# dexmal/dexbotic

Measured on AMD Instinct MI355X. Metric: episodes/sec DB-CogACT fine-tune, higher is better.
Workload: dtype bf16; 1 GPU; DB-CogACT fine-tune step (CLIP-L/14@224 x1 view, Qwen2.5-7B-class 28L decoder, DiT-B head, AdamW), 16 episodes/GPU, 32-token instruction, S=287; global_batch=16, seq_len=287, parallelism=dp1, optimizer=AdamW serial, grad_accum=1, activations=resident

## Files before the change

dexbotic_amd/_lib.py:

```python
from __future__ import annotations

import ctypes as C
import os

import torch

_HERE = os.path.dirname(os.path.abspath(__file__))
LIB_PATH = os.environ.get("DXA_LIB") or os.path.join(_HERE, "libdexbotic_amd.so")

F32, BF16 = 0, 1
ACT_NONE, ACT_GELU_ERF, ACT_GELU_TANH, ACT_QUICK_GELU, ACT_SILU, ACT_RELU, ACT_SIGMOID = 0, 1, 2, 3, 4, 5, 6
NT, NN, TN = 0, 1, 2
FILTER_BICUBIC = 3
FUSE_NONE, FUSE_SWIGLU = 0, 1

_vp, _i64, _i32, _f32, _sz = C.c_void_p, C.c_int64, C.c_int32, C.c_float, C.c_size_t
_int = C.c_int


class DxaError(RuntimeError):
    pass


class GemmDesc(C.Structure):
    _fields_ = [
        ("layout", _i32), ("in_dtype", _i32), ("out_dtype", _i32), ("act", _i32),
        ("M", _i64), ("N", _i64), ("K", _i64),
        ("A", _vp), ("lda", _i64), ("B", _vp), ("ldb", _i64), ("C", _vp), ("ldc", _i64),
        ("bias", _vp), ("residual", _vp), ("ldr", _i64), ("aux_out", _vp), ("mulgrad", _vp), ("ldg", _i64),
        ("alpha", _f32), ("accumulate", _i32), ("nb", _i32 * 3),
        ("sA", _i64 * 3), ("sB", _i64 * 3), ("sC", _i64 * 3), ("sR", _i64 * 3), ("sG", _i64 * 3),
        ("epi_f32", _i32), ("mirror", _vp), ("sumsq", _vp),
        ("A2", _vp), ("B2", _vp), ("K2", _i64),
        ("fuse", _i32), ("ld_aux", _i64),
    ]


class GemmStepInfo(C.Structure):
    _fields_ = [
        ("kernel", C.c_char_p), ("grid", _i32 * 3), ("block", _i32), ("lds", _i32),
        ("K", _i64), ("K2", _i64), ("a_off", _i64), ("b_off", _i64), ("seg2", _i32),
        ("accumulate", _i32), ("bias", _i32), ("residual", _i32),
        ("tm", _i32), ("tn", _i32), ("full", _i32), ("tail_r", _i32), ("split_s", _i32), ("group_m", _i32),
        ("vecA", _i32), ("vecB", _i32), ("vecC", _i32), ("vecR", _i32), ("vecG", _i32), ("vecBias", _i32),
        ("ksplit", _i32), ("kper", _i32), ("split_ws", _i32), ("mirror", _i32), ("sumsq", _i32),
    ]

# ... 32 lines not shown
        ("beta1", _f32), ("beta2", _f32), ("eps", _f32), ("bc1", _f32), ("bc2", _f32),
        ("clip_coef", _vp), ("g_dtype", _i32), ("chunk_state", _vp), ("chunk_mv_start", _vp),
    ]


class ImageDesc(C.Structure):
    _fields_ = [
        ("src", _vp), ("n", _i32), ("h", _i32), ("w", _i32), ("pad", _i32), ("bg", C.c_ubyte * 4),
        ("res_h", _i32), ("res_w", _i32), ("crop_top", _i32), ("crop_left", _i32), ("out_h", _i32), ("out_w", _i32),
        ("row0", _i32), ("rows", _i32), ("hb", _vp), ("hk", _vp), ("hks", _i32), ("vb", _vp), ("vk", _vp), ("vks", _i32),
        ("tmp", _vp), ("out", _vp), ("out_dtype", _i32), ("out_u8", _vp), ("rescale", C.c_double),
        ("mean", _f32 * 3), ("std", _f32 * 3),
    ]


class DecodeDesc(C.Structure):
    _fields_ = [
        ("layers", _vp), ("x_in", _vp), ("out", _vp), ("final_norm_w", _vp), ("cos_row", _vp), ("sin_row", _vp),
        ("workspace", _vp), ("workspace_bytes", _sz),
        ("n_layers", _i32), ("d", _i32), ("Hq", _i32), ("Hkv", _i32), ("D", _i32), ("F", _i32), ("slot", _i32), ("kv_lo", _i32),
        ("max_len", _i32), ("eps", _f32),
    ]


SIGNATURES = {
    "dxa_last_error": (C.c_char_p, []),
    "dxa_version": (_int, []),
    "dxa_gemm": (_int, [C.POINTER(GemmDesc), _vp]),
    "dxa_gemm_plan": (_int, [C.POINTER(GemmDesc), C.POINTER(GemmPlanInfo)]),
    "dxa_gemm_kernel_name": (C.c_char_p, [_int]),
    "dxa_split3": (_int, [_vp, _i64, _vp, _i64, _i64, _int, _vp]),
    "dxa_split3_t": (_int, [_vp, _i64, _vp, _i64, _i64, _i64, _int, _vp]),
    "dxa_split3_pair": (_int, [C.POINTER(Split3Op), C.POINTER(Split3Op), _vp]),
    "dxa_rmsnorm_fwd": (_int, [_vp, _vp, _vp, _vp, _i64, _i64, _f32, _int, _int, _vp]),
    "dxa_rmsnorm_bwd": (_int, [_vp, _vp, _vp, _vp, _vp, _vp, _vp, _i64, _i64, _int, _int, _vp]),
    "dxa_layernorm_fwd": (_int, [_vp, _vp, _vp, _vp, _vp, _vp, _i64, _i64, _f32, _int, _int, _vp]),
    "dxa_layernorm_bwd": (_int, [_vp, _vp, _vp, _vp, _vp, _vp, _vp, _vp, _i64, _i64, _int, _int, _vp]),
    "dxa_norm_bwd_blocks": (_int, [_i64]),
    "dxa_colsum": (_int, [_vp, _i64, _vp, _i64, _i64, _int, _int, _vp, _sz, _vp]),
    "dxa_rope_split": (_int, [_vp, _vp, _vp, _vp, _vp, _vp, _vp, _int, _int, _int, _int, _int, _int, _vp]),
    "dxa_rope_merge": (_int, [_vp, _vp, _vp, _vp, _vp, _vp, _vp, _int, _int, _int, _int, _int, _int, _vp]),
    "dxa_rope_split_at": (_int, [_vp, _vp, _vp, _vp, _vp, _vp, _vp, _int, _int, _int, _int, _int, _int, _int, _int, _vp]),
    "dxa_rope_merge_at": (_int, [_vp, _vp, _vp, _vp, _vp, _vp, _vp, _int, _int, _int, _int, _int, _int, _int, _int, _vp]),
    "dxa_attn_fwd": (_int, [C.POINTER(AttnDesc), _vp]),
    "dxa_attn_fwd_workspace": (_sz, [C.POINTER(AttnDesc)]),
    "dxa_attn_fwd_ws": (_int, [C.POINTER(AttnDesc), _vp, _sz, _vp]),
    "dxa_attn_bwd_workspace": (_sz, [C.POINTER(AttnDesc)]),
    "dxa_attn_bwd": (_int, [C.POINTER(AttnDesc), _vp, _sz, _vp]),
    "dxa_swiglu_fwd": (_int, [_vp, _vp, _i64, _i64, _int, _vp]),
    "dxa_swiglu_bwd": (_int, [_vp, _vp, _vp, _i64, _i64, _int, _vp]),
    "dxa_axpby": (_int, [_vp, _vp, _vp, _i64, _f32, _f32, _int, _vp]),
    "dxa_mul": (_int, [_vp, _vp, _vp, _i64, _int, _vp]),
    "dxa_mul_rows": (_int, [_vp, _vp, _vp, _i64, _i64, _i64, _int, _vp]),
    "dxa_glu_fwd": (_int, [_vp, _vp, _i64, _i64, _int, _int, _vp]),
    "dxa_glu_bwd": (_int, [_vp, _vp, _vp, _i64, _i64, _int, _int, _vp]),
    "dxa_act_fwd": (_int, [_vp, _vp, _i64, _int, _int, _vp]),
    "dxa_act_bwd": (_int, [_vp, _vp, _vp, _i64, _int, _int, _vp]),
    "dxa_add": (_int, [_vp, _vp, _vp, _i64, _int, _vp]),
    "dxa_cast": (_int, [_vp, _vp, _i64, _int, _int, _vp]),
    "dxa_copy2d": (_int, [_vp, _i64, _vp, _i64, _i64, _i64, _i64, _int, _int, _vp]),
    "dxa_transpose": (_int, [_vp, _i64, _vp, _i64, _i64, _i64, _i64, _int, _vp]),
    "dxa_permute_bshd": (_int, [_vp, _vp, _int, _int, _int, _int, _int, _int, _vp]),
    "dxa_splice_fwd": (_int, [_vp, _vp, _vp, _vp, _i64, _i64, _int, _vp]),
    "dxa_splice_bwd": (_int, [_vp, _vp, _vp, _vp, _i64, _i64, _int, _vp]),
    "dxa_zero_rows": (_int, [_vp, _vp, _i64, _i64, _vp]),
    "dxa_gather_rows": (_int, [_vp, _vp, _vp, _i64, _i64, _int, _int, _vp]),
# ... 77 lines not shown
```

dexbotic_amd/csrc/gemm.hip:

```cpp
#include "common.h"
#include "gemm_common.h"

#include <algorithm>
#include <cassert>

namespace {


template <typename T> struct EltTraits;
template <> struct EltTraits<float> { static constexpr int EPC = 4; };
template <> struct EltTraits<bf16_t> { static constexpr int EPC = 8; };

__device__ __forceinline__ int lds_off(int row, int chunk) { return row * ROWB + ((chunk ^ (row & 7)) << 4); }

template <typename T, int NR>
__device__ __forceinline__ void load_kc(uint4 (&r)[4], const T* __restrict__ base, int64_t ld, int64_t row0,
                                        int64_t rows, int64_t k0, int64_t K, int vec, int tid) {
  constexpr int EPC = EltTraits<T>::EPC;
  const int c = tid & 7;
  const int64_t k = k0 + (int64_t)c * EPC;
#pragma unroll
  for (int i = 0; i < NR / 32; ++i) {
    const int64_t row = row0 + (tid >> 3) + 32 * i;
    uint4 v = make_uint4(0, 0, 0, 0);
// ... 1213 lines not shown
  if (wm == 0) P3_BAR();
  P3_STAMP(2);
#undef P3_A_ROW0
#undef P3_B_ROW0
#undef P3_DMA
#undef P3_DMA_A
#undef P3_DMA_B
#undef P3_READ
#undef P3_RD_A
#undef P3_RD_B
#undef P3_MFMA
#undef P3_SB
#undef P3_BAR
#undef P3_COMPUTE
#undef P3_VMCNT
#undef P3_TILE
#undef P3_R_A1
#undef P3_R_A2B0
#undef P3_R_A0B1
  if constexpr (LEAN) {
    if (!tile_split_exchange<3>(p, acc, tid, split_j, split_s, tail_i)) return;
    __builtin_amdgcn_sched_barrier(0);
    if constexpr (FUSE == 1) sk_epilogue_swiglu<3>(p, acc, smem + wave * 4096, lane, wm, wn, (int)m0, (int)n0);
    else sk_epilogue<TO, TE, 3>(p, acc, smem + wave * 4096, lane, wm, wn, (int)m0, (int)n0, reinterpret_cast<float*>(smem + 8 * 4096), bid);
  } else {
    tile_finish<TO, 3, TE>(p, acc, smem, tid, lane, wave, wm, wn, l32, lh, m0, n0, split_j, split_s, tail_i);
  }
  asm volatile("s_waitcnt vmcnt(0)" ::: "memory");
  P3_STAMP(3);
#endif
}
#undef P3_STAMP

template <typename T>
__global__ __launch_bounds__(256) void sumsq_rows_k(const T* __restrict__ C, int64_t ldc, int64_t M, int64_t N,
                                                    float* __restrict__ out) {
  __shared__ float red[4];
  float s = 0.f;
  for (int64_t r = blockIdx.x; r < M; r += gridDim.x) {
    const T* row = C + r * ldc;
    for (int64_t c = threadIdx.x; c < N; c += 256) { const float v = ldf<T>(row + c); s += v * v; }
  }
#pragma unroll
  for (int o = 32; o > 0; o >>= 1) s += __shfl_xor(s, o, 64);
  if ((threadIdx.x & 63) == 0) red[threadIdx.x >> 6] = s;
  __syncthreads();
  if (threadIdx.x == 0) out[blockIdx.x] = (red[0] + red[1]) + (red[2] + red[3]);
}


constexpr int NUM_CU = 256;
static_assert(NUM_CU == NUM_CU_D, "split-K scratch sizing");
constexpr size_t SPLIT_WS_BYTES = (size_t)NUM_CU * 256 * 256 * 4;
int get_split_ws(hipStream_t st, char** ws) {
  static StreamBlock blocks(SPLIT_WS_BYTES + NUM_CU * sizeof(int));
  char* base = nullptr;
  if (int rc = blocks.get(st, &base)) return rc;
  DXA_CHECK_ARG(base != nullptr, "dxa_gemm: first split-K product on a stream allocates its scratch and cannot happen under stream "
                "capture: run the request once eagerly on this stream first");
  *ws = base;
  return DXA_OK;
}

enum GemmArgs { ARGS_P, ARGS_GEMV1, ARGS_GEMV2 };
struct GemmKernel {
  const char* name;
// ... 260 lines not shown
  p.C = (char*)d->C; p.ldc = d->ldc;
  p.bias = s.bias ? (const char*)d->bias : nullptr;
  p.R = s.residual ? (const char*)d->residual : nullptr; p.ldr = d->ldr;
  p.aux = (char*)d->aux_out;
  p.G = (const char*)d->mulgrad; p.ldg = d->ldg;
  p.alpha = d->alpha; p.act = d->act; p.accumulate = s.accumulate;
  p.fuse = d->fuse; p.ldaux = d->ld_aux;
  p.nb1 = d->nb[1]; p.nb2 = d->nb[2];
  for (int i = 0; i < 3; ++i) {
    p.sA[i] = d->sA[i]; p.sB[i] = d->sB[i]; p.sC[i] = d->sC[i]; p.sR[i] = d->sR[i]; p.sG[i] = d->sG[i];
  }
  p.tm = s.tm; p.tn = s.tn;
  p.vecA = s.vecA; p.vecB = s.vecB; p.vecC = s.vecC; p.vecR = s.vecR; p.vecG = s.vecG; p.vecBias = s.vecBias;
  p.full = s.full; p.tail_r = s.tail_r; p.split_s = s.split_s; p.group_m = s.group_m;
  if (s.mirror) p.mirror = (char*)d->mirror;
  if (s.sumsq) p.sumsq = d->sumsq;
  if (s.K2 > 0) { p.A2 = (const char*)d->A2; p.B2 = (const char*)d->B2; p.K2 = s.K2; }
  if (s.split_ws) {
    if (*ws == nullptr)
      if (int rc = get_split_ws(st, ws)) return rc;
    p.ws = (float*)*ws; p.flags = (int*)(*ws + SPLIT_WS_BYTES);
  }
  if (int rc = k.raise ? k.raise(k.lds) : DXA_OK) return rc;
  int M = (int)d->M, ksplit = s.ksplit, kper = s.kper;
  void* args_p[] = {&p};
  void* args_gemv1[] = {&p.A, &p.lda, &p.B, &p.ldb, &p.ws, &M, &p.N, &p.K, &kper};
  void* args_gemv2[] = {&p.ws, &p.C, &p.ldc, &M, &p.N, &ksplit, &p.alpha};
  void** args = k.args == ARGS_P ? args_p : k.args == ARGS_GEMV1 ? args_gemv1 : args_gemv2;
  (void)hipLaunchKernel(k.fn, dim3(s.grid[0], s.grid[1], s.grid[2]), dim3(k.block), args, k.lds, st);
  DXA_CHECK_LAUNCH();
  return DXA_OK;
}

}

extern "C" int64_t dxa_gemm_sumsq_slots(int64_t M, int64_t N) {
  if (M <= 0 || N <= 0) return 0;
  return ((M + 255) / 256) * ((N + 255) / 256);
}
extern "C" const char* dxa_gemm_kernel_name(int i) {
  return i >= 0 && i < NUM_KERNELS ? reinterpret_cast<const GemmKernel*>(&KERNELS)[i].name : nullptr;
}
extern "C" int dxa_gemm_plan(const dxa_gemm_desc* d, dxa_gemm_plan_info* out) {
  DXA_CHECK_ARG(out != nullptr, "dxa_gemm_plan: null output");
  GemmPlan plan;
  const int rc = gemm_plan(d, &plan);
  *out = plan.info;
  return rc;
}
extern "C" int dxa_gemm(const dxa_gemm_desc* d, dxa_stream_t stream) {
  GemmPlan plan;
  if (int rc = gemm_plan(d, &plan)) return rc;
  char* ws = nullptr;
  for (int i = 0; i < plan.info.nsteps; ++i) {
    if (int rc = gemm_run_step(d, plan.info.step[i], *plan.kernel[i], (hipStream_t)stream, &ws)) return rc;
  }
  if (plan.info.mirror_pass) {
    if (int rc = dxa_copy2d(d->C, d->ldc, d->mirror, d->ldc, d->M, d->N, d->N, DXA_F32, DXA_BF16, stream)) return rc;
  }
  if (plan.info.sumsq_pass) {
    const dim3 sgrid((unsigned)dxa_gemm_sumsq_slots(d->M, d->N));
    if (d->out_dtype == DXA_F32)
      hipLaunchKernelGGL(sumsq_rows_k<float>, sgrid, dim3(256), 0, (hipStream_t)stream, (const float*)d->C, d->ldc, d->M, d->N, d->sumsq);
    else
      hipLaunchKernelGGL(sumsq_rows_k<bf16_t>, sgrid, dim3(256), 0, (hipStream_t)stream, (const bf16_t*)d->C, d->ldc, d->M, d->N, d->sumsq);
    DXA_CHECK_LAUNCH();
  }
  return DXA_OK;
}

namespace {
struct S3Op { const float* src; int64_t ld; bf16_t* dst; int64_t rows, cols, pad; int side, transposed; unsigned nblocks, tiles_x; };
__global__ __launch_bounds__(256) void split3_pair_k(const S3Op a, const S3Op b) {
  __shared__ float tile[32][33];
  const bool first = blockIdx.x < a.nblocks;
  const S3Op& o = first ? a : b;
  const unsigned bid = first ? blockIdx.x : blockIdx.x - a.nblocks;
  if (!o.transposed) {
    const int64_t c4 = o.cols >> 2;
    for (int64_t i = (int64_t)bid * 256 + threadIdx.x; i < o.rows * c4; i += (int64_t)o.nblocks * 256) {
      const int64_t r = i / c4, c = (i - r * c4) * 4;
      float x[4];
      Vec<float, 4>::ld(x, o.src + r * o.ld + c);
      float hi[4], lo[4];
#pragma unroll
      for (int e = 0; e < 4; ++e) {
        hi[e] = bf2f(f2bf(x[e]));
        lo[e] = x[e] - hi[e];
      }
      bf16_t* d = o.dst + r * 3 * o.cols + c;
      Vec<bf16_t, 4>::st(d, hi);
      Vec<bf16_t, 4>::st(d + o.cols, o.side == 0 ? hi : lo);
      Vec<bf16_t, 4>::st(d + 2 * o.cols, o.side == 0 ? lo : hi);
    }
    return;
  }
  const int tx = threadIdx.x & 31, ty = threadIdx.x >> 5;
  const int64_t R = o.rows, C_ = o.cols, Rp = o.pad;
  const int64_t r0 = (int64_t)(bid / o.tiles_x) * 32, c0 = (int64_t)(bid % o.tiles_x) * 32;
#pragma unroll
  for (int i = 0; i < 4; ++i) {
// ... 75 lines not shown
```

dexbotic_amd/csrc/gemm_common.h:

```cpp
#pragma once
#include "common.h"

namespace dxa_gemm_detail {
typedef float f32x16_t __attribute__((ext_vector_type(16)));
struct GemmP {
  int64_t M, N, K;
  const char* A; int64_t lda;
  const char* B; int64_t ldb;
  char* C; int64_t ldc;
  const char* bias;
  const char* R; int64_t ldr;
  char* aux;
  const char* G; int64_t ldg;
  float alpha;
  int act, accumulate;
  int nb1, nb2;
  int64_t sA[3], sB[3], sC[3], sR[3], sG[3];
  int tm, tn;
  int vecA, vecB, vecC, vecR, vecG, vecBias;
  int full, tail_r, split_s;
  int group_m;
  char* mirror;
  float* sumsq;
  float* ws;
// ... 490 lines not shown
          const u32x2_t_ gv = {pack_bf16x2(g[0], g[1]), pack_bf16x2(g[2], g[3])};
          const u32x2_t_ uv = {pack_bf16x2(u[0], u[1]), pack_bf16x2(u[2], u[3])};
          __builtin_amdgcn_raw_buffer_store_b64(gv, rX, ok ? offG0 + rr * ldxB : 0x80000000u, 0, 0);
          __builtin_amdgcn_raw_buffer_store_b64(uv, rX, ok ? offU0 + rr * ldxB : 0x80000000u, 0, 0);
        }
      }
      __builtin_amdgcn_fence(__ATOMIC_RELEASE, "wavefront");
      __builtin_amdgcn_wave_barrier();
      __builtin_amdgcn_sched_barrier(0);
    }
#endif
}
template <typename TO, typename TE, int AI = 4, int MF = 32>
__device__ __forceinline__ void sk_epilogue(const GemmP& p, typename AccL<AI, MF>::T& acc, char* slab, int lane, int wm, int wn,
                                            int m0, int n0, float* red, int tile) {
#if defined(__HIP_DEVICE_COMPILE__)
  float ssq = sk_epilogue_rows<TO, TE, AI, MF>(p, acc, slab, lane, wm, wn, m0, n0);
  {
    if (p.sumsq != nullptr) {
#pragma unroll
      for (int o = 32; o > 0; o >>= 1) ssq += __shfl_xor(ssq, o, 64);
      if (lane == 0) red[wm * 4 + wn] = ssq;
      __syncthreads();
      if (threadIdx.x == 0) {
        float t = 0.f;
#pragma unroll
        for (int w8 = 0; w8 < 8; ++w8) t += red[w8];
        p.sumsq[tile] = t;
      }
    }
  }
#endif
}
}
```

dexbotic_amd/kernels.py:

```python
from __future__ import annotations

import contextlib
import ctypes as C
from typing import Optional, Sequence, Tuple

import torch

from . import _lib as L
from ._lib import lib

F32, BF16 = L.F32, L.BF16


def dt(t: torch.Tensor) -> int:
    if t.dtype == torch.float32:
        return F32
    if t.dtype == torch.bfloat16:
        return BF16
    raise L.DxaError(f"unsupported dtype {t.dtype} (fp32 / bf16 only)")


def torch_dtype(code: int) -> torch.dtype:
    return torch.bfloat16 if code == BF16 else torch.float32

# ... 52 lines not shown
    return out


def split3_pair(a: torch.Tensor, a_t: bool, b: torch.Tensor, b_t: bool, pad_to: int = 1, a_dims=None, b_dims=None
                ) -> Tuple[torch.Tensor, torch.Tensor]:
    ops, outs = [], []
    for x, t, side, dims in ((a, a_t, 0, a_dims), (b, b_t, 1, b_dims)):
        R, C_, ld = dims if dims is not None else (x.shape[0], x.shape[1], _row_major(x, "x"))
        o = L.Split3Op()
        o.src, o.ld, o.rows, o.cols, o.side, o.transposed = _ptr(x), ld, R, C_, side, int(t)
        if t:
            Rp = (R + pad_to - 1) // pad_to * pad_to
            out = torch.empty((C_, 3 * Rp), device=x.device, dtype=torch.bfloat16)
            o.pad = Rp
        else:
            out = torch.empty((R, 3 * C_), device=x.device, dtype=torch.bfloat16)
            o.pad = 0
        o.dst = _ptr(out)
        ops.append(o)
        outs.append(out)
    L.check(lib.dxa_split3_pair(C.byref(ops[0]), C.byref(ops[1]), _stream()), "dxa_split3_pair")
    return outs[0], outs[1]


def _x3_t_ok(M: int, N: int, Kc: int, out: torch.Tensor) -> bool:
    return (F32_GEMM_MODE == "bf16x3" and out.dtype == torch.float32 and M >= 128 and N >= 128 and Kc >= 64 and Kc % 32 == 0
            and 6 * max(M, N) * Kc < (1 << 31))


def mm_tn_f32(a: torch.Tensor, b: torch.Tensor, *, out: torch.Tensor, **kw) -> torch.Tensor:
    Kc, M = a.shape
    N = b.shape[1]
    if a.dtype == torch.float32 and b.dtype == torch.float32 and _x3_t_ok(M, N, (Kc + 31) // 32 * 32, out):
        a3, b3 = split3_pair(a, True, b, True, pad_to=32)
        Kp = a3.shape[1] // 3
        kw = _ld_kwargs(kw, out)
        return gemm(L.NT, a3, b3, M, N, 3 * Kp, 3 * Kp, 3 * Kp, out, _row_major(out, "out"), epi_f32=True, **kw)
    return mm_nt(transpose(a, 4), transpose(b, 4), out=out, **kw)


def mm_nn_f32(a: torch.Tensor, b: torch.Tensor, **kw) -> torch.Tensor:
    M, Kc = a.shape
    N = b.shape[1]
    out = kw.get("out")
    if (a.dtype == torch.float32 and b.dtype == torch.float32 and Kc % 32 == 0 and a.is_contiguous() and a.data_ptr() % 16 == 0
            and Kc % 4 == 0 and (out is None or out.dtype == torch.float32)):
        if out is None:
            out = kw["out"] = torch.empty((M, N), device=a.device, dtype=torch.float32)
        if _x3_t_ok(M, N, Kc, out):
            a3, b3 = split3_pair(a, False, b, True)
            kw2 = _ld_kwargs({k: v for k, v in kw.items() if k != "out"}, out)
            return gemm(L.NT, a3, b3, M, N, 3 * Kc, 3 * Kc, 3 * Kc, out, _row_major(out, "out"), epi_f32=True, **kw2)
    return mm_nt(a, transpose(b, 1), **kw)


def _x3_eligible(layout, a, b, out, M, N, K, lda, ldb, nb) -> bool:
    return (F32_GEMM_MODE == "bf16x3" and layout == L.NT and a.dtype == torch.float32 and b.dtype == torch.float32
            and out.dtype == torch.float32 and tuple(nb) == (1, 1, 1) and M >= 128 and N >= 128 and K >= 64 and K % 32 == 0
            and lda % 4 == 0 and ldb % 4 == 0 and a.data_ptr() % 16 == 0 and b.data_ptr() % 16 == 0
            and 6 * max(M, N) * K < (1 << 31))


_NB1 = (1, 1, 1)


def gemm(layout: int, a: torch.Tensor, b: torch.Tensor, M: int, N: int, K: int, lda: int, ldb: int,
         out: torch.Tensor, ldc: int, *, bias: Optional[torch.Tensor] = None,
         residual: Optional[torch.Tensor] = None, ldr: int = 0, act: int = L.ACT_NONE,
         aux_out: Optional[torch.Tensor] = None, mulgrad: Optional[torch.Tensor] = None, ldg: int = 0,
         alpha: float = 1.0, accumulate: bool = False, nb: Sequence[int] = _NB1,
         sA: Sequence[int] = (0, 0, 0), sB: Sequence[int] = (0, 0, 0), sC: Sequence[int] = (0, 0, 0),
         sR: Sequence[int] = (0, 0, 0), sG: Sequence[int] = (0, 0, 0), epi_f32: bool = False,
         mirror: Optional[torch.Tensor] = None, sumsq: Optional[torch.Tensor] = None,
         a2: Optional[torch.Tensor] = None, b2: Optional[torch.Tensor] = None) -> torch.Tensor:
    if not epi_f32 and a2 is None and _x3_eligible(layout, a, b, out, M, N, K, lda, ldb, nb):
        a3, b3 = split3_pair(a, False, b, False, a_dims=(M, K, lda), b_dims=(N, K, ldb))
        return gemm(L.NT, a3, b3, M, N, 3 * K, 3 * K, 3 * K, out, ldc, bias=bias, residual=residual, ldr=ldr, act=act,
                    aux_out=aux_out, mulgrad=mulgrad, ldg=ldg, alpha=alpha, accumulate=accumulate, epi_f32=True,
                    mirror=mirror, sumsq=sumsq)
    d = L.GemmDesc()
    d.layout, d.in_dtype, d.out_dtype, d.act = layout, dt(a), dt(out), act
    d.epi_f32 = int(epi_f32)
    if dt(b) != d.in_dtype:
        raise L.DxaError("gemm: A and B dtypes differ")
    for t, n in ((bias, "bias"), (residual, "residual"), (mulgrad, "mulgrad")):
        if t is not None and dt(t) != (F32 if epi_f32 else d.in_dtype):
            raise L.DxaError(f"gemm: {n} dtype must equal the input dtype")
    if aux_out is not None and dt(aux_out) != d.out_dtype:
        raise L.DxaError("gemm: aux_out dtype must equal the output dtype")
    d.M, d.N, d.K = M, N, K
    d.A, d.lda, d.B, d.ldb, d.C, d.ldc = _ptr(a), lda, _ptr(b), ldb, _ptr(out), ldc
    d.bias, d.residual, d.ldr = _ptr(bias), _ptr(residual), ldr
    d.aux_out, d.mulgrad, d.ldg = _ptr(aux_out), _ptr(mulgrad), ldg
    d.alpha, d.accumulate = alpha, int(accumulate)
    if mirror is not None:
        if mirror.dtype != torch.bfloat16 or out.dtype != torch.float32 or tuple(nb) != (1, 1, 1) or \
                _row_major(mirror, "mirror") != ldc:
            raise L.DxaError("gemm: mirror must be a bf16 [M, N] view with the output's leading dimension (fp32 output)")
        d.mirror = _ptr(mirror)
    if sumsq is not None:
        if sumsq.dtype != torch.float32 or tuple(nb) != (1, 1, 1) or not sumsq.is_contiguous() \
                or sumsq.numel() != gemm_sumsq_slots(M, N):
            raise L.DxaError("gemm: sumsq must be gemm_sumsq_slots(M, N) contiguous floats (unbatched output)")
        d.sumsq = _ptr(sumsq)
    if nb is _NB1 or tuple(nb) == (1, 1, 1):
        d.nb[0] = d.nb[1] = d.nb[2] = 1
    else:
        for i in range(3):
            d.nb[i], d.sA[i], d.sB[i], d.sC[i], d.sR[i], d.sG[i] = nb[i], sA[i], sB[i], sC[i], sR[i], sG[i]
    K_all = K
    if a2 is not None:
        if layout != L.TN or b2 is None or a2.shape[1] != M or b2.shape[1] != N or a2.shape[0] != b2.shape[0] \
                or dt(a2) != d.in_dtype or dt(b2) != d.in_dtype or _row_major(a2, "a2") != lda or _row_major(b2, "b2") != ldb:
            raise L.DxaError("gemm: a2 / b2 are a second [K2, M] / [K2, N] pair of a TN product (same dtypes and leading dimensions)")
        d.A2, d.B2, d.K2 = _ptr(a2), _ptr(b2), a2.shape[0]
        K_all = K + a2.shape[0]
    prof = GEMM_PROFILE
    if prof is not None and prof.wants(layout, d.in_dtype, d.out_dtype):
        e0, e1 = torch.cuda.Event(enable_timing=True), torch.cuda.Event(enable_timing=True)
        e0.record()
        L.check(lib.dxa_gemm(C.byref(d), _stream()), "dxa_gemm")
        e1.record()
        batches = nb[0] * nb[1] * nb[2]
        esz = {L.BF16: 2, L.F32: 4}
        prof.add((layout, d.in_dtype, d.out_dtype), e0, e1, 2.0 * M * N * K_all * batches,
                 float((M * K_all + N * K_all) * esz.get(d.in_dtype, 2) + M * N * esz.get(d.out_dtype, 2)) * batches)
        return out
    L.check(lib.dxa_gemm(C.byref(d), _stream()), "dxa_gemm")
    return out


class GemmProfile:

    def __init__(self, *keys, stride: int = 1):
        if len(keys) == 3 and all(isinstance(k, int) for k in keys):
            keys = (tuple(keys),)
        self.keys = set(tuple(k) for k in keys)
        self.events = []
        self.stride = max(1, int(stride))
        self.seen = {k: 0 for k in self.keys}

    def wants(self, layout, in_dtype, out_dtype) -> bool:
        key = (layout, in_dtype, out_dtype)
        if key not in self.keys:
            return False
        n = self.seen[key]
        self.seen[key] = n + 1
        return n % self.stride == 0

# ... 858 lines not shown
```

include/dexbotic_amd.h:

```cpp
#ifndef DEXBOTIC_AMD_H_
#define DEXBOTIC_AMD_H_

#include <stddef.h>
#include <stdint.h>

#ifdef __cplusplus
extern "C" {
#endif

typedef void* dxa_stream_t;

enum dxa_status { DXA_OK = 0, DXA_ERR_BAD_ARG = -1, DXA_ERR_UNSUPPORTED = -2, DXA_ERR_HIP = -3 };
enum dxa_dtype { DXA_F32 = 0, DXA_BF16 = 1 };
enum dxa_act {
  DXA_ACT_NONE = 0,
  DXA_ACT_GELU_ERF = 1,
  DXA_ACT_GELU_TANH = 2,
  DXA_ACT_QUICK_GELU = 3,
  DXA_ACT_SILU = 4,
  DXA_ACT_RELU = 5,
  DXA_ACT_SIGMOID = 6
};
enum dxa_layout {
  DXA_NT = 0,
// ... 40 lines not shown
int64_t dxa_gemm_sumsq_slots(int64_t M, int64_t N);
typedef struct dxa_gemm_step_info {
  const char* kernel;
  int32_t grid[3], block, lds;
  int64_t K, K2;
  int64_t a_off, b_off;
  int32_t seg2;
  int32_t accumulate, bias, residual;
  int32_t tm, tn, full, tail_r, split_s, group_m;
  int32_t vecA, vecB, vecC, vecR, vecG, vecBias;
  int32_t ksplit, kper;
  int32_t split_ws;
  int32_t mirror, sumsq;
} dxa_gemm_step_info;
typedef struct dxa_gemm_plan_info {
  int32_t nsteps;
  int32_t mirror_pass, sumsq_pass;
  dxa_gemm_step_info step[2];
} dxa_gemm_plan_info;
int dxa_gemm_plan(const dxa_gemm_desc* d, dxa_gemm_plan_info* out);
const char* dxa_gemm_kernel_name(int i);

int dxa_split3(const float* src, int64_t ld, void* dst, int64_t rows, int64_t cols, int side, dxa_stream_t stream);
int dxa_split3_t(const float* src, int64_t ld, void* dst, int64_t R, int64_t C, int64_t Rp, int side, dxa_stream_t stream);
typedef struct dxa_split3_op {
  const float* src;
  int64_t ld;
  void* dst;
  int64_t rows, cols, pad;
  int32_t side;
  int32_t transposed;
} dxa_split3_op;
int dxa_split3_pair(const dxa_split3_op* a, const dxa_split3_op* b, dxa_stream_t stream);

int dxa_rmsnorm_fwd(const void* x, const void* w, void* y, float* rstd, int64_t rows, int64_t cols,
                    float eps, int dtype, int w_dtype, dxa_stream_t stream);
int dxa_rmsnorm_bwd(const void* dy, const void* x, const void* w, const float* rstd, void* dx,
                    const void* residual, float* partial_dw, int64_t rows, int64_t cols, int dtype, int w_dtype,
                    dxa_stream_t stream);
int dxa_layernorm_fwd(const void* x, const void* w, const void* b, void* y, float* mean, float* rstd,
                      int64_t rows, int64_t cols, float eps, int dtype, int w_dtype, dxa_stream_t stream);
int dxa_layernorm_bwd(const void* dy, const void* x, const void* w, const float* mean, const float* rstd,
                      void* dx, const void* residual, float* partial_dwdb, int64_t rows, int64_t cols, int dtype,
                      int w_dtype, dxa_stream_t stream);
int dxa_norm_bwd_blocks(int64_t rows);
int dxa_colsum(const void* x, int64_t ld, float* out, int64_t rows, int64_t cols, int dtype,
               int accumulate, float* scratch, size_t scratch_bytes, dxa_stream_t stream);

int dxa_rope_split(const void* qkv, void* q, void* k, void* v, const float* cos_t, const float* sin_t,
                   const int32_t* pos, int B, int S, int Hq, int Hkv, int D, int dtype,
                   dxa_stream_t stream);
int dxa_rope_merge(const void* dq, const void* dk, const void* dv, void* dqkv, const float* cos_t,
                   const float* sin_t, const int32_t* pos, int B, int S, int Hq, int Hkv, int D,
                   int dtype, dxa_stream_t stream);
int dxa_rope_split_at(const void* qkv, void* q, void* k, void* v, const float* cos_t, const float* sin_t, const int32_t* pos, int B,
                      int S, int Hq, int Hkv, int D, int S_cap, int s0, int dtype, dxa_stream_t stream);
int dxa_rope_merge_at(const void* dq, const void* dk, const void* dv, void* dqkv, const float* cos_t, const float* sin_t,
                      const int32_t* pos, int B, int S, int Hq, int Hkv, int D, int S_cap, int s0, int dtype, dxa_stream_t stream);

typedef struct dxa_attn_desc {
  int32_t dtype;
  int32_t B, Hq, Hkv, Sq, Sk, D;
  int32_t causal;
  float scale;
  const void* q; int64_t q_sb, q_sh, q_ss;
  const void* k; int64_t k_sb, k_sh, k_ss;
// ... 180 lines not shown
```

Measured before the change: 71.27 episodes/s.

## Fuse fp32 bf16x3 split into a single GEMM kernel reading fp32 operands

Adds a dedicated gemm_x3 kernel that loads fp32 A/B tiles straight from global memory, splits them into bf16 hi/lo planes in LDS, and runs three MFMAs per tile pair (hi*hi, lo*hi, hi*lo). This replaces the previous path, which materialised split3 copies of both operands in global memory and then ran a 3K-long NT GEMM. The fp32 GEMM paths (TN, NN, and eligible NT) try the new kernel first and fall back to the old split path when it reports unsupported. The aim is to cut the extra memory traffic and launch of the split pass. The cost is a new, less-tuned kernel with fixed 64/128x64 tiles and no split-K.

```diff
diff --git a/dexbotic_amd/_lib.py b/dexbotic_amd/_lib.py
--- a/dexbotic_amd/_lib.py
+++ b/dexbotic_amd/_lib.py
@@ -13,6 +13,7 @@
 NT, NN, TN = 0, 1, 2
 FILTER_BICUBIC = 3
 FUSE_NONE, FUSE_SWIGLU = 0, 1
+OK, ERR_BAD_ARG, ERR_UNSUPPORTED, ERR_HIP = 0, -1, -2, -3
 
 _vp, _i64, _i32, _f32, _sz = C.c_void_p, C.c_int64, C.c_int32, C.c_float, C.c_size_t
 _int = C.c_int
@@ -111,6 +112,8 @@
     "dxa_split3": (_int, [_vp, _i64, _vp, _i64, _i64, _int, _vp]),
     "dxa_split3_t": (_int, [_vp, _i64, _vp, _i64, _i64, _i64, _int, _vp]),
     "dxa_split3_pair": (_int, [C.POINTER(Split3Op), C.POINTER(Split3Op), _vp]),
+    "dxa_gemm_x3": (_int, [C.POINTER(GemmDesc), _vp]),
+    "dxa_gemm_x3_plan": (_int, [C.POINTER(GemmDesc), C.POINTER(GemmPlanInfo)]),
     "dxa_rmsnorm_fwd": (_int, [_vp, _vp, _vp, _vp, _i64, _i64, _f32, _int, _int, _vp]),
     "dxa_rmsnorm_bwd": (_int, [_vp, _vp, _vp, _vp, _vp, _vp, _vp, _i64, _i64, _int, _int, _vp]),
     "dxa_layernorm_fwd": (_int, [_vp, _vp, _vp, _vp, _vp, _vp, _i64, _i64, _f32, _int, _int, _vp]),
diff --git a/dexbotic_amd/csrc/gemm.hip b/dexbotic_amd/csrc/gemm.hip
--- a/dexbotic_amd/csrc/gemm.hip
+++ b/dexbotic_amd/csrc/gemm.hip
@@ -1269,6 +1269,119 @@
 }
 #undef P3_STAMP
 
+template <int LAYOUT, int BM, bool RAG>
+__global__ __launch_bounds__(256) void gemm_x3_kernel(const GemmP p) {
+#if defined(__HIP_DEVICE_COMPILE__)
+  constexpr bool A_KS = LAYOUT == DXA_TN, B_KS = LAYOUT != DXA_NT;
+  constexpr int MI = BM / 32;
+  constexpr int A_PLANE = BM * X3_ROWB, B_PLANE = X3_BN * X3_ROWB;
+  constexpr int BUF = 2 * A_PLANE + 2 * B_PLANE;
+  __shared__ __attribute__((aligned(16))) char smem[2 * BUF];
+  const int tid = threadIdx.x, lane = tid & 63, wave = tid >> 6, wm = wave >> 1, wn = wave & 1;
+  const int pm = (int)blockIdx.x % p.tm, pn = (int)blockIdx.x / p.tm;
+  const int m0 = pm * BM, n0 = pn * X3_BN;
+  const int M = (int)p.M, N = (int)p.N, nk = (int)(p.K / X3_KS);
+  const uint32_t ldaB = (uint32_t)p.lda * 4u, ldbB = (uint32_t)p.ldb * 4u;
+  const int64_t bytesA = (A_KS ? (p.K - 1) * p.lda + p.M : (p.M - 1) * p.lda + p.K) * 4;
+  const int64_t bytesB = (B_KS ? (p.K - 1) * p.ldb + p.N : (p.N - 1) * p.ldb + p.K) * 4;
+  const __amdgpu_buffer_rsrc_t rA = __builtin_amdgcn_make_buffer_rsrc(const_cast<char*>(p.A), 0, (int)bytesA, 0x00020000);
+  const __amdgpu_buffer_rsrc_t rB = __builtin_amdgcn_make_buffer_rsrc(const_cast<char*>(p.B), 0, (int)bytesB, 0x00020000);
+
+  X3Stage<BM, A_KS, RAG> sa[4];
+  X3Stage<X3_BN, B_KS, RAG> sb[4];
+  f32x4_t acc[MI][2];
+#pragma unroll
+  for (int i = 0; i < MI; ++i)
+#pragma unroll
+    for (int j = 0; j < 2; ++j) acc[i][j] = (f32x4_t){0.f, 0.f, 0.f, 0.f};
+
+#define X3_LOAD(set, s) do { sa[set].load(rA, tid, m0, M, ldaB, (s) * X3_KS, (s) < nk); \
+                             sb[set].load(rB, tid, n0, N, ldbB, (s) * X3_KS, (s) < nk); } while (0)
+#define X3_STORE(set, buf) do { sa[set].store(smem + (buf) * BUF, smem + (buf) * BUF + A_PLANE, tid); \
+                                sb[set].store(smem + (buf) * BUF + 2 * A_PLANE, smem + (buf) * BUF + 2 * A_PLANE + B_PLANE, tid); } while (0)
+#define X3_BAR() do { __builtin_amdgcn_sched_barrier(0); asm volatile("s_waitcnt lgkmcnt(0)" ::: "memory"); \
+                      __builtin_amdgcn_s_barrier(); __builtin_amdgcn_sched_barrier(0); } while (0)
+  const int r16 = lane & 15, fc = lane >> 4;
+  auto compute = [&](int buf) {
+    const char* base = smem + buf * BUF;
+    bf16x8_t bh[2], bl[2];
+#pragma unroll
+    for (int j = 0; j < 2; ++j) {
+      const int r = wn * 32 + 16 * j + r16, o = r * X3_ROWB + x3_pos(r, fc) * 16;
+      bh[j] = *reinterpret_cast<const bf16x8_t*>(base + 2 * A_PLANE + o);
+      bl[j] = *reinterpret_cast<const bf16x8_t*>(base + 2 * A_PLANE + B_PLANE + o);
+    }
+#pragma unroll
+    for (int i = 0; i < MI; ++i) {
+      const int r = wm * (BM / 2) + 16 * i + r16, o = r * X3_ROWB + x3_pos(r, fc) * 16;
+      const bf16x8_t ah = *reinterpret_cast<const bf16x8_t*>(base + o);
+      const bf16x8_t al = *reinterpret_cast<const bf16x8_t*>(base + A_PLANE + o);
+#pragma unroll
+      for (int j = 0; j < 2; ++j) {
+        acc[i][j] = __builtin_amdgcn_mfma_f32_16x16x32_bf16(bh[j], ah, acc[i][j], 0, 0, 0);
+        acc[i][j] = __builtin_amdgcn_mfma_f32_16x16x32_bf16(bl[j], ah, acc[i][j], 0, 0, 0);
+        acc[i][j] = __builtin_amdgcn_mfma_f32_16x16x32_bf16(bh[j], al, acc[i][j], 0, 0, 0);
+      }
+    }
+  };
+
+  X3_LOAD(0, 0);
+  X3_LOAD(1, 1);
+  X3_LOAD(2, 2);
+  X3_LOAD(3, 3);
+  X3_STORE(0, 0);
+  X3_BAR();
+  for (int s = 0; s < nk; s += 4) {
+    X3_LOAD(0, s + 4);
+    compute(0);
+    X3_STORE(1, 1);
+    X3_BAR();
+    X3_LOAD(1, s + 5);
+    compute(1);
+    X3_STORE(2, 0);
+    X3_BAR();
+    X3_LOAD(2, s + 6);
+    compute(0);
+    X3_STORE(3, 1);
+    X3_BAR();
+    X3_LOAD(3, s + 7);
+    compute(1);
+    X3_STORE(0, 0);
+    X3_BAR();
+  }
+#undef X3_LOAD
+#undef X3_STORE
+#undef X3_BAR
+
+  float* C = reinterpret_cast<float*>(p.C);
+  float* AUX = p.aux ? reinterpret_cast<float*>(p.aux) : nullptr;
+  const float* R = reinterpret_cast<const float*>(p.R);
+  const float* G = reinterpret_cast<const float*>(p.G);
+  const float* bias = reinterpret_cast<const float*>(p.bias);
+  bf16_t* mirror = reinterpret_cast<bf16_t*>(p.mirror);
+#pragma unroll
+  for (int j = 0; j < 2; ++j) {
+    const int64_t n = n0 + wn * 32 + 16 * j + 4 * fc;
+    const int n_ok = (int)max((int64_t)0, min((int64_t)4, p.N - n));
+    if (n_ok <= 0) continue;
+    float bv[4] = {0.f, 0.f, 0.f, 0.f};
+    if (bias) load4<float>(bv, bias + n, p.vecBias, n_ok);
+#pragma unroll
+    for (int i = 0; i < MI; ++i) {
+      const int64_t m = m0 + wm * (BM / 2) + 16 * i + r16;
+      if (m >= p.M) continue;
+      const float a4[4] = {acc[i][j][0], acc[i][j][1], acc[i][j][2], acc[i][j][3]};
+      epilogue4<float, float>(p, C, AUX, R, G, bv, m, n, n_ok, a4);
+      if (mirror) {
+        float c4[4];
+        load4<float>(c4, C + m * p.ldc + n, p.vecC, n_ok);
+        store4<bf16_t>(mirror + m * p.ldc + n, c4, p.vecC, n_ok);
+      }
+    }
+  }
+#endif
+}
+
 template <typename T>
 __global__ __launch_bounds__(256) void sumsq_rows_k(const T* __restrict__ C, int64_t ldc, int64_t M, int64_t N,
                                                     float* __restrict__ out) {
@@ -1595,29 +1708,58 @@
   return DXA_OK;
 }
 
-}
-
-extern "C" int64_t dxa_gemm_sumsq_slots(int64_t M, int64_t N) {
-  if (M <= 0 || N <= 0) return 0;
-  return ((M + 255) / 256) * ((N + 255) / 256);
-}
-extern "C" const char* dxa_gemm_kernel_name(int i) {
-  return i >= 0 && i < NUM_KERNELS ? reinterpret_cast<const GemmKernel*>(&KERNELS)[i].name : nullptr;
-}
-extern "C" int dxa_gemm_plan(const dxa_gemm_desc* d, dxa_gemm_plan_info* out) {
-  DXA_CHECK_ARG(out != nullptr, "dxa_gemm_plan: null output");
-  GemmPlan plan;
-  const int rc = gemm_plan(d, &plan);
-  *out = plan.info;
-  return rc;
-}
-extern "C" int dxa_gemm(const dxa_gemm_desc* d, dxa_stream_t stream) {
-  GemmPlan plan;
-  if (int rc = gemm_plan(d, &plan)) return rc;
-  char* ws = nullptr;
-  for (int i = 0; i < plan.info.nsteps; ++i) {
-    if (int rc = gemm_run_step(d, plan.info.step[i], *plan.kernel[i], (hipStream_t)stream, &ws)) return rc;
-  }
+constexpr int x3_lds(int bm) { return 2 * (2 * bm * X3_ROWB + 2 * X3_BN * X3_ROWB); }
+constexpr int X3_LDS_LIMIT = 65536;
+static_assert(x3_lds(128) <= X3_LDS_LIMIT, "gemm_x3_kernel keeps its tiles in default-size LDS");
+#define KROW_X3_1(LAYOUT, BM, RAG, n) GemmKernel{n, reinterpret_cast<const void*>(gemm_x3_kernel<LAYOUT, BM, RAG>), 256, 0, nullptr, ARGS_P}
+#define KROW_X3(LAYOUT, RAG, l) {{KROW_X3_1(LAYOUT, 64, false, "x3<" l ",64>"), KROW_X3_1(LAYOUT, 128, false, "x3<" l ",128>")}, \
+                                 {KROW_X3_1(LAYOUT, 64, RAG, "x3<" l ",64,ragged>"), KROW_X3_1(LAYOUT, 128, RAG, "x3<" l ",128,ragged>")}}
+const GemmKernel X3_KERNELS[3][2][2] = {KROW_X3(DXA_NT, false, "nt"), KROW_X3(DXA_NN, true, "nn"), KROW_X3(DXA_TN, true, "tn")};
+
+int gemm_x3_plan(const dxa_gemm_desc* d, GemmPlan* plan) {
+  memset(plan, 0, sizeof(*plan));
+  DXA_CHECK_ARG(d != nullptr, "dxa_gemm_x3: null desc");
+  DXA_CHECK_ARG(d->M >= 0 && d->N >= 0 && d->K >= 0, "dxa_gemm_x3: negative dims");
+  DXA_CHECK_ARG(d->layout >= DXA_NT && d->layout <= DXA_TN, "dxa_gemm_x3: bad layout %d", d->layout);
+  DXA_CHECK_ARG(d->nb[0] >= 1 && d->nb[1] >= 1 && d->nb[2] >= 1, "dxa_gemm_x3: batch extents must be >= 1");
+#define X3_NEEDS(cond, ...) do { if (!(cond)) { dxa_set_error(__VA_ARGS__); return DXA_ERR_UNSUPPORTED; } } while (0)
+  X3_NEEDS(d->in_dtype == DXA_F32 && d->out_dtype == DXA_F32 && !d->epi_f32, "dxa_gemm_x3: fp32 operands and output only");
+  X3_NEEDS(d->nb[0] * d->nb[1] * d->nb[2] == 1 && d->fuse == DXA_FUSE_NONE && d->K2 == 0 && !d->A2 && !d->B2,
+           "dxa_gemm_x3: one unbatched, unfused product without a second segment");
+  X3_NEEDS(d->M >= 1 && d->N >= 1 && d->K >= X3_KS && d->K % X3_KS == 0, "dxa_gemm_x3: K must be a positive multiple of %d (K = %lld)",
+           X3_KS, (long long)d->K);
+  DXA_CHECK_ARG(d->A && d->B && d->C, "dxa_gemm_x3: null operand");
+  const bool a_ks = d->layout == DXA_TN, b_ks = d->layout != DXA_NT;
+  X3_NEEDS(aligned_to(d->A, 16) && aligned_to(d->B, 16) && d->lda % 4 == 0 && d->ldb % 4 == 0 &&
+           d->lda >= (a_ks ? d->M : d->K) && d->ldb >= (b_ks ? d->N : d->K), "dxa_gemm_x3: operand rows must be 16-byte aligned");
+  const int64_t bytesA = (a_ks ? (d->K - 1) * d->lda + d->M : (d->M - 1) * d->lda + d->K) * 4;
+  const int64_t bytesB = (b_ks ? (d->K - 1) * d->ldb + d->N : (d->N - 1) * d->ldb + d->K) * 4;
+  X3_NEEDS(bytesA < (1ll << 31) && bytesB < (1ll << 31), "dxa_gemm_x3: operands must be smaller than 2 GiB");
+#undef X3_NEEDS
+  dxa_gemm_step_info s;
+  memset(&s, 0, sizeof(s));
+  s.K = d->K;
+  s.accumulate = d->accumulate; s.bias = d->bias != nullptr; s.residual = d->residual != nullptr;
+  s.vecA = s.vecB = 1;
+  s.vecC = aligned_to(d->C, 16) && d->ldc % 4 == 0 && (!d->aux_out || aligned_to(d->aux_out, 16));
+  s.vecR = d->residual && aligned_to(d->residual, 16) && d->ldr % 4 == 0;
+  s.vecG = d->mulgrad && aligned_to(d->mulgrad, 16) && d->ldg % 4 == 0;
+  s.vecBias = d->bias && aligned_to(d->bias, 16);
+  const bool big = (int64_t)dxa_cdiv(d->M, 128) * dxa_cdiv(d->N, X3_BN) >= 192;
+  const int bm = big ? 128 : 64;
+  s.tm = dxa_cdiv(d->M, bm); s.tn = dxa_cdiv(d->N, X3_BN);
+  DXA_CHECK_ARG((int64_t)s.tm * s.tn < (1ll << 31), "dxa_gemm_x3: too many tiles");
+  s.full = s.tm * s.tn; s.split_s = 1;
+  s.mirror = d->mirror && (!s.vecC || aligned_to(d->mirror, 8));
+  const bool ragged = (a_ks && d->M % 4 != 0) || (b_ks && d->N % 4 != 0);
+  plan_add(plan, s, X3_KERNELS[d->layout][ragged][big], (int64_t)s.tm * s.tn);
+  plan->info.step[0].lds = x3_lds(bm);
+  plan->info.mirror_pass = d->mirror && !s.mirror;
+  plan->info.sumsq_pass = d->sumsq != nullptr;
+  return DXA_OK;
+}
+
+int gemm_post_passes(const dxa_gemm_desc* d, const GemmPlan& plan, dxa_stream_t stream) {
   if (plan.info.mirror_pass) {
     if (int rc = dxa_copy2d(d->C, d->ldc, d->mirror, d->ldc, d->M, d->N, d->N, DXA_F32, DXA_BF16, stream)) return rc;
   }
@@ -1630,6 +1772,46 @@
     DXA_CHECK_LAUNCH();
   }
   return DXA_OK;
+}
+
+}
+
+extern "C" int64_t dxa_gemm_sumsq_slots(int64_t M, int64_t N) {
+  if (M <= 0 || N <= 0) return 0;
+  return ((M + 255) / 256) * ((N + 255) / 256);
+}
+extern "C" const char* dxa_gemm_kernel_name(int i) {
+  return i >= 0 && i < NUM_KERNELS ? reinterpret_cast<const GemmKernel*>(&KERNELS)[i].name : nullptr;
+}
+extern "C" int dxa_gemm_plan(const dxa_gemm_desc* d, dxa_gemm_plan_info* out) {
+  DXA_CHECK_ARG(out != nullptr, "dxa_gemm_plan: null output");
+  GemmPlan plan;
+  const int rc = gemm_plan(d, &plan);
+  *out = plan.info;
+  return rc;
+}
+extern "C" int dxa_gemm(const dxa_gemm_desc* d, dxa_stream_t stream) {
+  GemmPlan plan;
+  if (int rc = gemm_plan(d, &plan)) return rc;
+  char* ws = nullptr;
+  for (int i = 0; i < plan.info.nsteps; ++i) {
+    if (int rc = gemm_run_step(d, plan.info.step[i], *plan.kernel[i], (hipStream_t)stream, &ws)) return rc;
+  }
+  return gemm_post_passes(d, plan, stream);
+}
+extern "C" int dxa_gemm_x3_plan(const dxa_gemm_desc* d, dxa_gemm_plan_info* out) {
+  DXA_CHECK_ARG(out != nullptr, "dxa_gemm_x3_plan: null output");
+  GemmPlan plan;
+  const int rc = gemm_x3_plan(d, &plan);
+  *out = plan.info;
+  return rc;
+}
+extern "C" int dxa_gemm_x3(const dxa_gemm_desc* d, dxa_stream_t stream) {
+  GemmPlan plan;
+  if (int rc = gemm_x3_plan(d, &plan)) return rc;
+  char* ws = nullptr;
+  if (int rc = gemm_run_step(d, plan.info.step[0], *plan.kernel[0], (hipStream_t)stream, &ws)) return rc;
+  return gemm_post_passes(d, plan, stream);
 }
 
 namespace {
diff --git a/dexbotic_amd/csrc/gemm_common.h b/dexbotic_amd/csrc/gemm_common.h
--- a/dexbotic_amd/csrc/gemm_common.h
+++ b/dexbotic_amd/csrc/gemm_common.h
@@ -546,4 +546,82 @@
   }
 #endif
 }
-}
+
+constexpr int X3_KS = 32;
+constexpr int X3_ROWB = 2 * X3_KS;
+constexpr int X3_BN = 64;
+constexpr uint32_t X3_OOB = 0x80000000u;
+__device__ __forceinline__ int x3_pos(int r, int c) { return c ^ ((0 - (r >> 2)) & 3); }
+__device__ __forceinline__ void x3_split4(float x0, float x1, float x2, float x3, uint32_t (&hi)[2], uint32_t (&lo)[2]) {
+  hi[0] = pack_bf16x2(x0, x1);
+  hi[1] = pack_bf16x2(x2, x3);
+  lo[0] = pack_bf16x2(x0 - __uint_as_float(hi[0] << 16), x1 - __uint_as_float(hi[0] & 0xffff0000u));
+  lo[1] = pack_bf16x2(x2 - __uint_as_float(hi[1] << 16), x3 - __uint_as_float(hi[1] & 0xffff0000u));
+}
+__device__ __forceinline__ f32x4_t x3_ld16(__amdgpu_buffer_rsrc_t r, uint32_t off) {
+  return __builtin_bit_cast(f32x4_t, __builtin_amdgcn_raw_buffer_load_b128(r, off, 0, 0));
+}
+__device__ __forceinline__ f32x4_t x3_ld_ragged(__amdgpu_buffer_rsrc_t r, uint32_t off, int n_ok) {
+  f32x4_t v;
+#pragma unroll
+  for (int e = 0; e < 4; ++e)
+    v[e] = __uint_as_float(__builtin_amdgcn_raw_buffer_load_b32(r, e < n_ok ? off + 4u * e : X3_OOB, 0, 0));
+  return v;
+}
+
+template <int ROWS, bool KS, bool RAG = false> struct X3Stage;
+template <int ROWS, bool RAG> struct X3Stage<ROWS, false, RAG> {
+  static constexpr int NI = ROWS * 4 / 256;
+  f32x4_t v[NI][2];
+  __device__ __forceinline__ void load(__amdgpu_buffer_rsrc_t rs, int tid, int row0, int rows, uint32_t ldB, int k0, bool k_ok) {
+#pragma unroll
+    for (int i = 0; i < NI; ++i) {
+      const int id = tid + 256 * i, r = id >> 2, c = id & 3;
+      const bool ok = k_ok && row0 + r < rows;
+      const uint32_t off = ok ? (uint32_t)(row0 + r) * ldB + (uint32_t)(k0 + c * 8) * 4u : X3_OOB;
+      v[i][0] = x3_ld16(rs, off);
+      v[i][1] = x3_ld16(rs, off + 16u);
+    }
+  }
+  __device__ __forceinline__ void store(char* hi_plane, char* lo_plane, int tid) const {
+#pragma unroll
+    for (int i = 0; i < NI; ++i) {
+      const int id = tid + 256 * i, r = id >> 2, c = id & 3;
+      uint32_t h0[2], l0[2], h1[2], l1[2];
+      x3_split4(v[i][0][0], v[i][0][1], v[i][0][2], v[i][0][3], h0, l0);
+      x3_split4(v[i][1][0], v[i][1][1], v[i][1][2], v[i][1][3], h1, l1);
+      const int o = r * X3_ROWB + x3_pos(r, c) * 16;
+      *reinterpret_cast<uint4*>(hi_plane + o) = make_uint4(h0[0], h0[1], h1[0], h1[1]);
+      *reinterpret_cast<uint4*>(lo_plane + o) = make_uint4(l0[0], l0[1], l1[0], l1[1]);
+    }
+  }
+};
+template <int ROWS, bool RAG> struct X3Stage<ROWS, true, RAG> {
+  static constexpr int CNT = 2 * ROWS;
+  f32x4_t v[4];
+  __device__ __forceinline__ void load(__amdgpu_buffer_rsrc_t rs, int tid, int col0, int cols, uint32_t ldB, int k0, bool k_ok) {
+    const int kg = tid & 7, n = col0 + 4 * (tid >> 3), n_ok = cols - n;
+    const bool ok = k_ok && n_ok > 0 && tid < CNT;
+#pragma unroll
+    for (int j = 0; j < 4; ++j) {
+      const uint32_t off = ok ? (uint32_t)(k0 + kg * 4 + j) * ldB + (uint32_t)n * 4u : X3_OOB;
+      if constexpr (RAG) v[j] = x3_ld_ragged(rs, off, ok ? n_ok : 0);
+      else v[j] = x3_ld16(rs, off);
+    }
+  }
+  __device__ __forceinline__ void store(char* hi_plane, char* lo_plane, int tid) const {
+    if (tid < CNT) {
+      const int kg = tid & 7, ng = tid >> 3;
+#pragma unroll
+      for (int e = 0; e < 4; ++e) {
+        const int r = 4 * ng + e;
+        uint32_t h[2], l[2];
+        x3_split4(v[0][e], v[1][e], v[2][e], v[3][e], h, l);
+        const int o = r * X3_ROWB + x3_pos(r, kg >> 1) * 16 + (kg & 1) * 8;
+        *reinterpret_cast<uint2*>(hi_plane + o) = make_uint2(h[0], h[1]);
+        *reinterpret_cast<uint2*>(lo_plane + o) = make_uint2(l[0], l[1]);
+      }
+    }
+  }
+};
+}
diff --git a/dexbotic_amd/kernels.py b/dexbotic_amd/kernels.py
--- a/dexbotic_amd/kernels.py
+++ b/dexbotic_amd/kernels.py
@@ -108,9 +108,11 @@
     Kc, M = a.shape
     N = b.shape[1]
     if a.dtype == torch.float32 and b.dtype == torch.float32 and _x3_t_ok(M, N, (Kc + 31) // 32 * 32, out):
+        kw = _ld_kwargs(kw, out)
+        if gemm_x3(L.TN, a, b, M, N, Kc, _row_major(a, "a"), _row_major(b, "b"), out, _row_major(out, "out"), **kw):
+            return out
         a3, b3 = split3_pair(a, True, b, True, pad_to=32)
         Kp = a3.shape[1] // 3
-        kw = _ld_kwargs(kw, out)
         return gemm(L.NT, a3, b3, M, N, 3 * Kp, 3 * Kp, 3 * Kp, out, _row_major(out, "out"), epi_f32=True, **kw)
     return mm_nt(transpose(a, 4), transpose(b, 4), out=out, **kw)
 
@@ -124,8 +126,10 @@
         if out is None:
             out = kw["out"] = torch.empty((M, N), device=a.device, dtype=torch.float32)
         if _x3_t_ok(M, N, Kc, out):
+            kw2 = _ld_kwargs({k: v for k, v in kw.items() if k != "out"}, out)
+            if gemm_x3(L.NN, a, b, M, N, Kc, _row_major(a, "a"), _row_major(b, "b"), out, _row_major(out, "out"), **kw2):
+                return out
             a3, b3 = split3_pair(a, False, b, True)
-            kw2 = _ld_kwargs({k: v for k, v in kw.items() if k != "out"}, out)
             return gemm(L.NT, a3, b3, M, N, 3 * Kc, 3 * Kc, 3 * Kc, out, _row_major(out, "out"), epi_f32=True, **kw2)
     return mm_nt(a, transpose(b, 1), **kw)
 
@@ -140,20 +144,8 @@
 _NB1 = (1, 1, 1)
 
 
-def gemm(layout: int, a: torch.Tensor, b: torch.Tensor, M: int, N: int, K: int, lda: int, ldb: int,
-         out: torch.Tensor, ldc: int, *, bias: Optional[torch.Tensor] = None,
-         residual: Optional[torch.Tensor] = None, ldr: int = 0, act: int = L.ACT_NONE,
-         aux_out: Optional[torch.Tensor] = None, mulgrad: Optional[torch.Tensor] = None, ldg: int = 0,
-         alpha: float = 1.0, accumulate: bool = False, nb: Sequence[int] = _NB1,
-         sA: Sequence[int] = (0, 0, 0), sB: Sequence[int] = (0, 0, 0), sC: Sequence[int] = (0, 0, 0),
-         sR: Sequence[int] = (0, 0, 0), sG: Sequence[int] = (0, 0, 0), epi_f32: bool = False,
-         mirror: Optional[torch.Tensor] = None, sumsq: Optional[torch.Tensor] = None,
-         a2: Optional[torch.Tensor] = None, b2: Optional[torch.Tensor] = None) -> torch.Tensor:
-    if not epi_f32 and a2 is None and _x3_eligible(layout, a, b, out, M, N, K, lda, ldb, nb):
-        a3, b3 = split3_pair(a, False, b, False, a_dims=(M, K, lda), b_dims=(N, K, ldb))
-        return gemm(L.NT, a3, b3, M, N, 3 * K, 3 * K, 3 * K, out, ldc, bias=bias, residual=residual, ldr=ldr, act=act,
-                    aux_out=aux_out, mulgrad=mulgrad, ldg=ldg, alpha=alpha, accumulate=accumulate, epi_f32=True,
-                    mirror=mirror, sumsq=sumsq)
+def _gemm_desc(layout, a, b, M, N, K, lda, ldb, out, ldc, bias, residual, ldr, act, aux_out, mulgrad, ldg, alpha, accumulate,
+               nb, sA, sB, sC, sR, sG, epi_f32, mirror, sumsq, a2, b2):
     d = L.GemmDesc()
     d.layout, d.in_dtype, d.out_dtype, d.act = layout, dt(a), dt(out), act
     d.epi_f32 = int(epi_f32)
@@ -191,6 +183,39 @@
             raise L.DxaError("gemm: a2 / b2 are a second [K2, M] / [K2, N] pair of a TN product (same dtypes and leading dimensions)")
         d.A2, d.B2, d.K2 = _ptr(a2), _ptr(b2), a2.shape[0]
         K_all = K + a2.shape[0]
+    return d, K_all
+
+
+def gemm_x3(layout: int, a: torch.Tensor, b: torch.Tensor, M: int, N: int, K: int, lda: int, ldb: int, out: torch.Tensor, ldc: int,
+            *, bias=None, residual=None, ldr: int = 0, act: int = L.ACT_NONE, aux_out=None, mulgrad=None, ldg: int = 0,
+            alpha: float = 1.0, accumulate: bool = False, mirror=None, sumsq=None) -> bool:
+    d, _ = _gemm_desc(layout, a, b, M, N, K, lda, ldb, out, ldc, bias, residual, ldr, act, aux_out, mulgrad, ldg, alpha, accumulate,
+                      _NB1, None, None, None, None, None, False, mirror, sumsq, None, None)
+    rc = lib.dxa_gemm_x3(C.byref(d), _stream())
+    if rc == L.ERR_UNSUPPORTED:
+        return False
+    L.check(rc, "dxa_gemm_x3")
+    return True
+
+
+def gemm(layout: int, a: torch.Tensor, b: torch.Tensor, M: int, N: int, K: int, lda: int, ldb: int,
+         out: torch.Tensor, ldc: int, *, bias: Optional[torch.Tensor] = None,
+         residual: Optional[torch.Tensor] = None, ldr: int = 0, act: int = L.ACT_NONE,
+         aux_out: Optional[torch.Tensor] = None, mulgrad: Optional[torch.Tensor] = None, ldg: int = 0,
+         alpha: float = 1.0, accumulate: bool = False, nb: Sequence[int] = _NB1,
+         sA: Sequence[int] = (0, 0, 0), sB: Sequence[int] = (0, 0, 0), sC: Sequence[int] = (0, 0, 0),
+         sR: Sequence[int] = (0, 0, 0), sG: Sequence[int] = (0, 0, 0), epi_f32: bool = False,
+         mirror: Optional[torch.Tensor] = None, sumsq: Optional[torch.Tensor] = None,
+         a2: Optional[torch.Tensor] = None, b2: Optional[torch.Tensor] = None) -> torch.Tensor:
+    if not epi_f32 and a2 is None and _x3_eligible(layout, a, b, out, M, N, K, lda, ldb, nb):
+        epi = dict(bias=bias, residual=residual, ldr=ldr, act=act, aux_out=aux_out, mulgrad=mulgrad, ldg=ldg, alpha=alpha,
+                   accumulate=accumulate, mirror=mirror, sumsq=sumsq)
+        if gemm_x3(L.NT, a, b, M, N, K, lda, ldb, out, ldc, **epi):
+            return out
+        a3, b3 = split3_pair(a, False, b, False, a_dims=(M, K, lda), b_dims=(N, K, ldb))
+        return gemm(L.NT, a3, b3, M, N, 3 * K, 3 * K, 3 * K, out, ldc, epi_f32=True, **epi)
+    d, K_all = _gemm_desc(layout, a, b, M, N, K, lda, ldb, out, ldc, bias, residual, ldr, act, aux_out, mulgrad, ldg, alpha, accumulate,
+                          nb, sA, sB, sC, sR, sG, epi_f32, mirror, sumsq, a2, b2)
     prof = GEMM_PROFILE
     if prof is not None and prof.wants(layout, d.in_dtype, d.out_dtype):
         e0, e1 = torch.cuda.Event(enable_timing=True), torch.cuda.Event(enable_timing=True)
diff --git a/include/dexbotic_amd.h b/include/dexbotic_amd.h
--- a/include/dexbotic_amd.h
+++ b/include/dexbotic_amd.h
@@ -96,6 +96,8 @@
   int32_t transposed;
 } dxa_split3_op;
 int dxa_split3_pair(const dxa_split3_op* a, const dxa_split3_op* b, dxa_stream_t stream);
+int dxa_gemm_x3(const dxa_gemm_desc* d, dxa_stream_t stream);
+int dxa_gemm_x3_plan(const dxa_gemm_desc* d, dxa_gemm_plan_info* out);
 
 int dxa_rmsnorm_fwd(const void* x, const void* w, void* y, float* rstd, int64_t rows, int64_t cols,
                     float eps, int dtype, int w_dtype, dxa_stream_t stream);
```

After: 70.52 episodes/s. 1.1% lower.
